# GuyTevet/motion-diffusion-model

Measured on AMD Instinct MI355X. Metric: motions/sec (B=128, T=196, 50-step DDPM), higher is better.
Workload: dtype f16x3 (fp32 operands split into fp16 hi+lo, 3 fp16 MFMA products, fp32 accumulate; everything else fp32); 1 GPU; HumanML3D text2motion, 50-step p_sample_loop with CFG 2.5 (2 denoiser forwards per step), batch=128 per GPU, T=196, 8-layer d=512 trans_enc MDM, random-init weights, cached text embedding; global_batch=128, diffusion_steps=50, parallelism=dp1: batch shards, no data-path collective, all_gather of final samples

## Files before the change

include/mdm_hip.h:

```cpp
#ifndef MDM_HIP_H
#define MDM_HIP_H

#include <stddef.h>
#include <stdint.h>

#ifdef __cplusplus
extern "C" {
#endif

#define MDM_OK 0
#define MDM_EINVAL (-1)
#define MDM_ESTATE (-2)
#define MDM_ENOSPC (-3)
#define MDM_EHIP (-4)
#define MDM_EUNSUPPORTED (-5)

#define MDM_ABI_VERSION 10

typedef struct mdm_model mdm_model_t;

#define MDM_ARCH_TRANS_ENC 0
#define MDM_ARCH_TRANS_DEC 1

typedef struct mdm_config {
// ... 12 lines not shown

int mdm_abi_version(void);
const char* mdm_build_info(void);
const char* mdm_last_error(void);

int mdm_create(const mdm_config_t* cfg, mdm_model_t** out);
void mdm_destroy(mdm_model_t* m);

#define MDM_OPT_SMALL_GEMM_MAX_SEQS 1
#define MDM_OPT_SMALL_GEMM_ROW_TILES 2
#define MDM_OPT_DEC_FUSED_XATTN 3
#define MDM_OPT_DEC_FUSED_SELFATTN 4
#define MDM_OPT_ATTN_DIRECT_OUT 5
#define MDM_OPT_DEC_TIME_TOKEN 6
#define MDM_OPT_ENC_SHARED_LAYER0 7
int mdm_set_option(mdm_model_t* m, int32_t key, int32_t value);
int mdm_get_option(const mdm_model_t* m, int32_t key, int32_t* value);

int mdm_set_time_add(mdm_model_t* m, const float* add_dev, int32_t B);

int mdm_set_weight(mdm_model_t* m, const char* name, const float* dev_ptr, int64_t numel);

size_t mdm_const_bytes(const mdm_model_t* m);
int mdm_prepare(mdm_model_t* m, void* const_ws_dev, size_t const_ws_bytes, void* stream);

int mdm_weights_in_range(mdm_model_t* m, int32_t* in_range, void* stream);

#define MDM_PREC_F32 0
#define MDM_PREC_F16X3 1
int mdm_set_precision(mdm_model_t* m, int32_t mode);
// ... 171 lines not shown
```

motion-diffusion-model_amd/_native.py:

```python
import ctypes as C
import os

_HERE = os.path.dirname(os.path.abspath(__file__))
LIB_NAME = "libmdm_hip.so"
LIB_PATH = os.path.join(_HERE, "csrc", LIB_NAME)
PROBE_LIB_PATH = os.path.join(_HERE, "csrc", "libmdm_hip_probe.so")

MDM_OK = 0
BRANCH_COND, BRANCH_UNCOND, BRANCH_BOTH = 0, 1, 2
ACT_NONE, ACT_GELU, ACT_SILU = 0, 1, 2
PRECISIONS = {"f32": 0, "f16x3": 1}
PROF_CLASSES = ("linear", "attention", "layernorm", "embed", "outproj", "elementwise")

EXPORTED_SYMBOLS = [
    "mdm_abi_version", "mdm_build_info", "mdm_last_error", "mdm_create", "mdm_destroy", "mdm_set_weight", "mdm_const_bytes",
    "mdm_prepare", "mdm_workspace_bytes", "mdm_forward", "mdm_sampler_step", "mdm_randn", "mdm_sample_loop",
    "mdm_linear", "mdm_layernorm", "mdm_attention", "mdm_profile_enable", "mdm_profile_read", "mdm_profile_reset",
    "mdm_set_precision", "mdm_linear_x3", "mdm_linear_x3_scratch_bytes", "mdm_attention_x3", "mdm_attention_x3_scratch_bytes",
    "mdm_recover_from_ric", "mdm_workspace_bytes_dec", "mdm_forward_dec", "mdm_workspace_bytes_dec_loop",
    "mdm_sample_loop_dec", "mdm_weights_in_range", "mdm_set_option", "mdm_get_option", "mdm_set_time_add",
    "mdm_rot6d_to_smpl_joints", "mdm_smpl_workspace_bytes", "mdm_smpl_forward",
    "mdm_eval_workspace_bytes", "mdm_eval_motion_embeddings", "mdm_eval_text_embeddings",
]
PROBE_SYMBOLS = ["mdm_debug_set", "mdm_debug_get", "mdm_linear_f16f6", "mdm_linear_f16f6_scratch_bytes", "mdm_probe_in_proj"]
ABI_VERSION = 10
OPTIONS = {"small_gemm_max_seqs": 1, "small_gemm_row_tiles": 2, "dec_fused_xattn": 3, "dec_fused_selfattn": 4, "attn_direct_out": 5,
           "dec_time_token": 6, "enc_shared_layer0": 7}
ARCH = {"trans_enc": 0, "trans_dec": 1}


class MdmConfig(C.Structure):
    _fields_ = [(n, C.c_int32) for n in ("njoints", "nfeats", "latent_dim", "ff_size", "num_layers", "num_heads",
                                         "clip_dim", "max_len", "mask_frames", "arch", "context_len")]


class MdmSmplModel(C.Structure):
    _fields_ = [(n, C.c_void_p) for n in ("j0", "jdirs", "blend", "weights_t", "sel_blend", "sel_weights_t", "extra_t")] + \
               [("parents", C.POINTER(C.c_int32))] + [(n, C.c_int32) for n in ("J", "V", "n_sel", "n_extra")]


class MdmSmplCall(C.Structure):
    _fields_ = [(n, C.c_int32) for n in ("pose_rep", "glob", "translation", "vertstrans", "n_points", "root_point")] + \
# ... 149 lines not shown
```

motion-diffusion-model_amd/csrc/api_launch.h:

```cpp
#pragma once

namespace {

struct Workspace {
  float *tok, *qkv, *att, *ffn, *cond;
  QkvPlanes qp;
  p16_t *xah, *xal;
  float *stat1, *stat2;
  p16_t *tokh, *tokl;
  p16_t *atth, *attl;
  p16_t *ffnh, *ffnl;
  size_t bytes;
};

QkvPlanes carve_qkv_planes(float* qkv, size_t nseq, size_t S, size_t D, int H) {
  const size_t NKT = (S + 31) / 32, SP = 32 * NKT, plane = nseq * SP * D;
  p16_t* q = reinterpret_cast<p16_t*>(qkv);
  QkvPlanes qp{};
  qp.qh = q; qp.SP = (int)SP; qp.NKT = (int)NKT; qp.H = H;
  if (q != nullptr) { qp.ql = q + plane; qp.kh = q + 2 * plane; qp.kl = q + 3 * plane; qp.vh = q + 4 * plane; qp.vl = q + 5 * plane; }
  return qp;
}

Workspace carve(const mdm_model* m, int nseq, int T, void* base) {
// ... 125 lines not shown
struct X3Call {
  X3Kind kind = X3K_OUT_LN_RES;
  Profiler* pf = nullptr; int prof_cat = MDM_PROF_LINEAR;
  X3Operand a{nullptr, nullptr}; X3Weights w{nullptr, nullptr}; const float* bias = nullptr;
  float* out = nullptr; p16_t* oh = nullptr; p16_t* ol = nullptr; const QkvPlanes* qp = nullptr;
  int M = 0, N = 0, K = 0, S = 0, D = 0;
  int scale_cols = 0; float col_scale = 1.f;
  const float* astat = nullptr; const float* colsum = nullptr;
  X3Operand res{nullptr, nullptr}; const float* rstat = nullptr; const float* rgamma = nullptr; const float* rbeta = nullptr;
  float* ostat = nullptr;
  int parts = 1; float inv_dim = 1.f;
  const float* res_f32 = nullptr; int emb_T = 1, emb_B = 1, emb_nbranch = 1;
  bool small = false;
  X3sShape shape{1};
  int stat_cols = 256;
};
X3Epilogue x3_epilogue(const X3Call& c) {
  X3Epilogue ep{};
  ep.out = c.out; ep.bias = c.bias; ep.res = c.res_f32; ep.resh = c.res.hi; ep.resl = c.res.lo; ep.oh = c.oh; ep.ol = c.ol;
  ep.ld = c.N; ep.scale_cols = c.scale_cols; ep.col_scale = c.col_scale;
  if (c.qp != nullptr) ep.qkv = *c.qp;
  ep.S = c.S; ep.D = c.D;
  ep.astat = c.astat; ep.colsum = c.colsum; ep.rstat = c.rstat; ep.rgamma = c.rgamma; ep.rbeta = c.rbeta; ep.ostat = c.ostat;
  ep.stat_parts = c.parts; ep.inv_dim = c.inv_dim; ep.emb_T = c.emb_T; ep.emb_B = c.emb_B; ep.emb_nbranch = c.emb_nbranch;
  ep.stat_cols = c.stat_cols;
  return ep;
}

#ifdef MDM_PROBES
int g_f6_linear = 0;
// ... 105 lines not shown
  const X3Epilogue ep = x3_epilogue(c);
  const bool in_proj = kind == X3K_IN_PROJ_FOLD || kind == X3K_IN_PROJ_PLAIN;
  if (c.small) {
    const int group_rows = in_proj ? S : (kind == X3K_EMBED ? c.emb_T : M);
    const int rc = launch_gemm_x3s(kind, c.shape, c.a, c.w, ep, M, N, K, group_rows, s);
    if (rc == -1 || rc == -3) return lds_fail(rc, "f16x3 linear (small tiles)");
    if (rc == -2) return fail(MDM_EUNSUPPORTED, "f16x3 linear (small tiles): unsupported shape (K must be 288 or a multiple of 256)");
    return rt_launch_status();
  }
  if (kind == X3K_IN_PROJ_PLAIN) {
    const int rc6 = launch_gemm_x3_qkv(c.a, c.w, ep, M / S, S, c.D, s);
    if (rc6 != 0) return fail(MDM_EUNSUPPORTED, "f16x3 in_proj: launch failed");
    return rt_launch_status();
  }
  const int rpt = (kind == X3K_IN_PROJ_FOLD) ? S : x3_rows_per_tile(M, kind == X3K_EMBED ? c.emb_T : S);
  const int rc = launch_gemm_x3_ln(kind, c.a, c.w, ep, M, N, K, rpt, s);
  if (rc == -1 || rc == -3) return lds_fail(rc, "f16x3 linear");
  if (rc == -2) return fail(MDM_EUNSUPPORTED, "f16x3 linear: unsupported folded-LayerNorm GEMM kind");
  return rt_launch_status();
}

int launch_pack_weights(const float* src, p16_t* hi, p16_t* lo, int N, int K, hipStream_t s, int* overflow = nullptr) {
  if (K % 16 != 0) return fail(MDM_EINVAL, "pack_weights: K must be a multiple of 16");
  const size_t n = x3_packed_weight_elems(N, K) / 8;
  const int grid = (int)std::min<size_t>((n + 255) / 256, 4096);
  MDM_LAUNCH(pack_weight_planes_kernel, dim3(grid), dim3(256), 0, s, src, hi, lo, N, K, overflow);
  return rt_launch_status();
}

int launch_split(const float* src, p16_t* hi, p16_t* lo, size_t n, hipStream_t s) {
  if (n % 4 != 0) return fail(MDM_EINVAL, "split: element count must be a multiple of 4");
// ... 8 lines not shown
```

motion-diffusion-model_amd/csrc/api_runtime.h:

```cpp
#pragma once

namespace {

thread_local std::string g_err;
#ifdef MDM_PROBES
int g_x3_reuse_planes = 0;
int g_f6_reference = 0;
#else
constexpr int g_x3_reuse_planes = 0;
#endif

int fail(int code, const std::string& msg) {
  g_err = msg;
  return code;
}

#ifdef MDM_EMU
inline int rt_launch_status() { return 0; }
inline int rt_copy(void* dst, const void* src, size_t bytes, hipStream_t) { memcpy(dst, src, bytes); return 0; }
template <class K> inline int rt_allow_lds(K, size_t) { return 0; }
#else
inline int rt_launch_status() {
  hipError_t e = hipGetLastError();
  if (e != hipSuccess) return fail(MDM_EHIP, std::string("kernel launch failed: ") + hipGetErrorString(e));
// ... 105 lines not shown
  std::vector<LayerFold> fold;
  struct DecFold { float *w_in, *c_in, *b_in, *w_q, *c_q, *b_q, *w_1, *c_1, *b_1; };
  std::vector<DecFold> dec_fold;
  struct DecPlanes { X3Weights in_proj, out_proj, q, out_proj2, linear1, linear2; };
  std::vector<DecPlanes> dec_planes;
  X3Weights in_planes{nullptr, nullptr};
  int jf_k = 0;
  X3Weights out_planes_f{nullptr, nullptr};
  float *c_out = nullptr, *b_out = nullptr;
  float *wkv_all = nullptr, *bkv_all = nullptr;
  bool lnfold = false;
  X3sOptions x3s;
  int fused_xattn = 3;
  bool fused_selfattn = true;
  bool enc_shared_l0 = true;
  bool attn_direct = false;
  X3Weights out_planes{nullptr, nullptr};
  float* out_bias_pad = nullptr;
  int jf_out = 0;

  const float* W(const std::string& k) const { return w.at(k); }
  const float* L(int layer, const char* suffix) const {
    return w.at((cfg.arch == MDM_ARCH_TRANS_DEC ? "seqTransDecoder.layers." : "seqTransEncoder.layers.") +
                std::to_string(layer) + "." + suffix);
  }
};

namespace {

#ifdef MDM_EMU
// ... 65 lines not shown
```

motion-diffusion-model_amd/csrc/common.h:

```cpp
#pragma once
#ifdef MDM_EMU
#include "hip_emu.h"
#else
#include <hip/hip_runtime.h>
#define MDM_DYN_SMEM(type, name) \
  extern __shared__ __attribute__((aligned(16))) unsigned char mdm_dyn_smem_raw[]; \
  type* name = reinterpret_cast<type*>(mdm_dyn_smem_raw)
#define MDM_LAUNCH(kernel, grid, block, shmem, stream, ...) \
  hipLaunchKernelGGL(kernel, (grid), (block), (shmem), (stream), __VA_ARGS__)
#endif
#include <stdint.h>
#include <type_traits>
#include <utility>

namespace mdm {

typedef float f32x16 __attribute__((ext_vector_type(16)));
typedef short p16x8 __attribute__((ext_vector_type(8)));

constexpr int kWave = 64;

constexpr int kMaxDevices = 64;
inline int rt_device_ordinal() {
#ifdef MDM_EMU
// ... 112 lines not shown
  return __shfl_xor(v, mask, 64);
#endif
}

__device__ __forceinline__ float sum_lanes8(float v) {
#ifdef MDM_EMU
  v += shfl_xor_f32(v, 1);
  v += shfl_xor_f32(v, 2);
  v += shfl_xor_f32(v, 4);
  return v;
#else
  v += __builtin_bit_cast(float, __builtin_amdgcn_update_dpp(0, __builtin_bit_cast(int, v), 0xB1, 0xF, 0xF, true));
  v += __builtin_bit_cast(float, __builtin_amdgcn_update_dpp(0, __builtin_bit_cast(int, v), 0x4E, 0xF, 0xF, true));
  v += __builtin_bit_cast(float, __builtin_amdgcn_update_dpp(0, __builtin_bit_cast(int, v), 0x141, 0xF, 0xF, true));
  return v;
#endif
}

template <int KT>
__device__ __forceinline__ bool key_valid_bits(const uint32_t* __restrict__ w, int row, int lead) {
  const int f = row - lead;
  uint32_t word;
  if (f >= 0) word = w[KT];
  else word = (KT > 0) ? w[KT > 0 ? KT - 1 : 0] : 0xffffffffu;
  return (word >> (f & 31)) & 1u;
}

__device__ __forceinline__ float4 ld4(const float* p) { return *reinterpret_cast<const float4*>(p); }
__device__ __forceinline__ void st4(float* p, float4 v) { *reinterpret_cast<float4*>(p) = v; }
__device__ __forceinline__ float4 zero4() { return make_float4(0.f, 0.f, 0.f, 0.f); }
// ... 215 lines not shown
  split2_p16(v.x, v.y, h01, l01);
  split2_p16(v.z, v.w, h23, l23);
  clip_store8(hi_w, off, u32x2{h01, h23});
  clip_store8(lo_w, off, u32x2{l01, l23});
}
__device__ __forceinline__ void clip_load8_async(u32x2& dst, const ClipWin& w, uint32_t off) {
#ifdef MDM_EMU
  static const uint32_t zeros[2] = {0u, 0u};
  const bool in = off < w.bytes && off + 8 <= w.bytes;
  emu::vm_issue(&dst, in ? static_cast<const void*>(w.base + off) : static_cast<const void*>(zeros), 8, true);
#else
  asm volatile("buffer_load_dwordx2 %0, %1, %2, 0 offen" : "=&v"(dst) : "v"(off), "s"(w.d) : "memory");
#endif
}

__device__ __forceinline__ void wg_barrier() {
#ifdef MDM_EMU
  emu::lgkm_wait(0);
  emu::block_barrier();
#else
  __builtin_amdgcn_s_waitcnt(0xC07F);
  __builtin_amdgcn_s_barrier();
#endif
}
__device__ __forceinline__ void wg_barrier_nodrain() {
#ifdef MDM_EMU
  emu::block_barrier();
#else
  __builtin_amdgcn_s_barrier();
#endif
// ... 79 lines not shown
```

motion-diffusion-model_amd/csrc/decoder.h:

```cpp
#pragma once

namespace {
struct DecWorkspace {
  float *tok, *qkv, *att, *ffn, *mem, *kv, *proj;
  float *stat[2];
  p16_t *xh[2], *xl[2];
  p16_t *atth, *attl, *ffnh, *ffnl;
  QkvPlanes qp;
  float *out;
  float *kv_text;
  float *kv_time;
  float *time_rows;
  float *o_text;
  float *o_time;
  size_t bytes;
};
DecWorkspace carve_dec(const mdm_model* m, int nseq, int S, int ntok, int B, void* base, int nsteps = 0, int pred_len = 0) {
  const size_t D = m->cfg.latent_dim, FF = m->cfg.ff_size, M = (size_t)nseq * S, Mm = (size_t)nseq * ntok;
  size_t off = 0;
  auto take = [&](size_t floats) {
    size_t o = off;
    off += align_up(floats * sizeof(float), 256);
    return base ? reinterpret_cast<float*>(static_cast<char*>(base) + o) : nullptr;
  };
// ... 128 lines not shown

struct DecLayer {
  int l; p16_t *Xh, *Xl, *Yh, *Yl; float *sX, *sY;
  X3Operand X() const { return X3Operand{Xh, Xl}; }
  X3Operand Y() const { return X3Operand{Yh, Yl}; }
};
struct DecStack {
  mdm_model_t* m; const DecWorkspace& ws; const DecHoist& hz; hipStream_t s; Profiler* pf;
  const int32_t* text_lengths; const int32_t* len;
  int B, nbranch, nseq, S, ntok, D, H, FF, M;
  bool small; X3sShape shape; int scols, parts; float inv_dim, qscale;

  X3Call LN(X3Kind kind, X3Operand a, X3Weights w, const float* bias, int rows, int N, int K) const {
    X3Call c; c.kind = kind; c.pf = pf; c.a = a; c.w = w; c.bias = bias; c.M = rows; c.N = N; c.K = K; c.S = S; c.D = D;
    c.small = small; c.shape = shape; c.stat_cols = scols; c.parts = parts; c.inv_dim = inv_dim;
    return c;
  }
  SelfAttnArgs seqhead_args() const {
    SelfAttnArgs a{};
    a.qscale = qscale; a.lead = 0; a.B = B; a.oh = ws.atth; a.ol = ws.attl;
    a.M = M; a.S = S; a.D = D; a.H = H; a.stat_parts = parts; a.stat_cols = scols; a.inv_dim = inv_dim; a.acc_scale = kX3AccScale;
    return a;
  }

  int self_attention(const DecLayer& y, DecSelfForm form, bool share0) const {
    const int l = y.l;
    const mdm_model::DecFold& F = m->dec_fold[l];
    const mdm_model::DecPlanes& P = m->dec_planes[l];
    const int M0 = (share0 && l == 0) ? B * S : M;
    const float* b_in = l == 0 ? m->L(l, "self_attn.in_proj_bias") : F.b_in;
// ... 258 lines not shown
```

motion-diffusion-model_amd/csrc/encoder.h:

```cpp
#pragma once

namespace {

int embed_frames_x3(mdm_model* m, const Workspace& ws, const float* x, int B, int T, int nbranch, hipStream_t s, const CondTokArgs& ct) {
  const int D = m->cfg.latent_dim, KP = m->jf_k;
  ProfScope ps(&m->prof, MDM_PROF_EMBED, 2.0 * B * T * (double)D * m->jf, s);
  p16_t* ph = reinterpret_cast<p16_t*>(ws.ffn);
  p16_t* pl = ph + (size_t)B * T * KP;
  MDM_LAUNCH(pose_planes_cond_kernel, dim3(((T + 31) / 32) * (KP / 32) * B + nbranch * B), dim3(256), 0, s, x, ph, pl, T, m->jf, KP, B, ct);
  if (int rc = rt_launch_status()) return rc;
  X3Call c;
  c.kind = X3K_EMBED; c.prof_cat = MDM_PROF_EMBED;
  c.a = X3Operand{ph, pl}; c.w = m->in_planes; c.bias = m->W("input_process.poseEmbedding.bias");
  c.oh = ws.tokh; c.ol = ws.tokl; c.M = B * T; c.N = D; c.K = KP; c.S = T + 1; c.D = D;
  c.res_f32 = m->W("sequence_pos_encoder.pe");
  c.emb_T = T; c.emb_B = B; c.emb_nbranch = nbranch;
  c.small = use_small_gemm(m, nbranch * B, T + 1) && KP == 288;
  c.shape = x3s_shape(m->x3s, nbranch * B);
  return launch_x3_ln(c, s);
}
inline bool use_embed_x3(const mdm_model* m, int T) {
  return m->precision == MDM_PREC_F16X3 &&
         (T + 1 <= X3_TM || (use_small_gemm(m, 1, T + 1) && m->jf_k == 288));
}
// ... 22 lines not shown
                                false, s)) return rc;
  ProfScope ps(&m->prof, MDM_PROF_ELEMENTWISE, 0.0, s);
  MDM_LAUNCH(cond_token_kernel, dim3(nbranch * B), dim3(128), 0, s, ws.tok, cond_emb, m->W("embed_text.bias"),
             (const float*)m->time_table, timesteps, t_uniform, m->W("sequence_pos_encoder.pe"), B, S, D, uncond_from_branch,
             (int)m->cfg.max_len, x3 ? ws.tokh : (p16_t*)nullptr, x3 ? ws.tokl : (p16_t*)nullptr, m->time_add);
  return rt_launch_status();
}

X3Call enc_ln_call(mdm_model* m, int nseq, int S) {
  const int D = m->cfg.latent_dim;
  X3Call c; c.M = nseq * S; c.S = S; c.D = D; c.inv_dim = 1.0f / (float)D;
  c.small = use_small_gemm(m, nseq, S);
  c.shape = x3s_shape(m->x3s, nseq);
  c.stat_cols = c.small ? X3S_TN : 256;
  c.parts = (D + c.stat_cols - 1) / c.stat_cols;
  return c;
}

int encoder(mdm_model* m, const Workspace& ws, int nseq, int B, int S, const int* lengths, hipStream_t s) {
  Profiler* pf = &m->prof;
  const int D = m->cfg.latent_dim, FF = m->cfg.ff_size, H = m->cfg.num_heads, M = nseq * S;
  const float qscale = 1.0f / sqrtf((float)(D / H));
  if (m->precision == MDM_PREC_F16X3 && m->lnfold && (S <= X3_TM || use_small_gemm(m, nseq, S))) {
    const X3Operand xb{ws.tokh, ws.tokl}, xa{ws.xah, ws.xal}, attp{ws.atth, ws.attl}, ffnp{ws.ffnh, ws.ffnl};
    const X3Call stack = enc_ln_call(m, nseq, S);
    const bool small = stack.small;
    auto LN = [&](X3Kind kind, X3Operand a, X3Weights w, const float* bias, int N, int K) {
      X3Call c = stack; c.kind = kind; c.pf = pf; c.a = a; c.w = w; c.bias = bias; c.N = N; c.K = K;
      return c;
    };
// ... 96 lines not shown
```

motion-diffusion-model_amd/csrc/gemm_x3.h:

```cpp
#pragma once
#include "attention_x3.h"
#include "common.h"
#include "gemm_f32.h"

namespace mdm {

constexpr int X3_TM = 224, X3_BK = 32;
__host__ __device__ constexpr int x3_swz(int q) { return (((q ^ (q >> 1)) & 1) << 1) | (q >> 1); }
static_assert(x3_swz(0) == 0 && x3_swz(1) == 2 && x3_swz(2) == 3 && x3_swz(3) == 1, "A-stage swizzle permutation");
constexpr int X3_NWAVE = 8;
constexpr int X3_TN = 32 * X3_NWAVE;
constexpr int X3_MSUB = X3_TM / 32;
constexpr int X3_A_BYTES = X3_TM * X3_BK * 2;
constexpr int X3_A_STAGE = 2 * X3_A_BYTES;
constexpr int X3_A_RING = 2;
constexpr int X3_PIPE_RING = 4;
constexpr int X3M_WAIT_WS = 7, X3M_WAIT_MID = 11;
constexpr int x3_patch_base(int ring) { return ring * X3_A_STAGE; }
constexpr int X3_PATCH_BYTES = 8 * 32 * 4;
constexpr int X3_TAB_BYTES = X3_TM * 8;
constexpr int x3_tab_base(int ring) { return x3_patch_base(ring) + X3_NWAVE * X3_PATCH_BYTES; }
constexpr int X3_RAW_BYTES = 7 * 1024;
constexpr int x3_raw_base(int ring) { return x3_tab_base(ring) + 2 * X3_TAB_BYTES; }
constexpr int x3_part_base(int ring) { return x3_raw_base(ring) + 2 * X3_RAW_BYTES; }
// ... 104 lines not shown
  int k;
  uint32_t off[X3_A_PIECES];
};

enum : unsigned {
  X3_OUT_F32 = 1u << 0,
  X3_OUT_PLANES = 1u << 1,
  X3_OUT_QKV = 1u << 2,
  X3_FOLD = 1u << 3,
  X3_OSTAT = 1u << 4,
  X3_EMBED = 1u << 5,
  X3_T16 = 1u << 6,
  X3_F6 = 1u << 7,
  X3_PIPE = 1u << 8,
  X3_PAIR = 1u << 9,
};
template <int ACT, int RES, unsigned FLAGS>
__global__ __launch_bounds__(64 * X3_NWAVE, 2) void gemm_x3_kernel(X3Operand A, X3Weights W, X3Epilogue ep, int M, int N, int K,
                                                                   int rows_per_tile, int tiles_n, int total) {
  MDM_DYN_SMEM(unsigned char, lds);
  constexpr bool OUT_F32 = (FLAGS & X3_OUT_F32) != 0, OUT_PLANES = (FLAGS & X3_OUT_PLANES) != 0, OUT_QKV = (FLAGS & X3_OUT_QKV) != 0;
  constexpr bool FOLD = (FLAGS & X3_FOLD) != 0, OSTAT = (FLAGS & X3_OSTAT) != 0, EMBED = (FLAGS & X3_EMBED) != 0;
  constexpr bool T16 = (FLAGS & X3_T16) != 0, F6 = (FLAGS & X3_F6) != 0, PIPE = (FLAGS & X3_PIPE) != 0, PAIR = (FLAGS & X3_PAIR) != 0;
  static_assert(FLAGS < (X3_PAIR << 1), "unknown flag");
  static_assert((int)OUT_F32 + (int)OUT_PLANES + (int)OUT_QKV == 1, "exactly one output form");
  static_assert(RES >= 0 && RES <= 3 && !(OUT_QKV && RES != 0), "in_proj has no residual");
  static_assert(!(FOLD && RES == 3), "one (mean, rstd) table: of the A rows or of the residual rows");
  static_assert(!OSTAT || OUT_PLANES, "row statistics are written next to the planes they describe");
  static_assert(!EMBED || (OUT_PLANES && RES == 1 && !PIPE), "InputProcess: fp32 positional rows, planes out, step-synchronous loop");
  static_assert(!PIPE || (T16 && !F6), "the pipelined k-loop exists for 208-row (T16) tiles");
  static_assert(!F6 || (!T16 && OUT_F32 && !FOLD && !OSTAT), "the f16f6 k-loop: 224-row tiles, plain fp32-out epilogues");
  static_assert(!PAIR || (PIPE && OUT_QKV && !FOLD), "the paired tile: layer 0's in_proj (no folded LayerNorm) on the pipelined loop");
  constexpr int RINGN = PIPE ? X3_PIPE_RING : X3_A_RING;
  constexpr int NT32 = T16 ? X3_MSUB - 1 : X3_MSUB;
  constexpr int NROUNDS = 4 * NT32 + (T16 ? 2 : 0);
  using Cursor = X3Cursor;

  const int tid = threadIdx.x;
  const int lane = tid & 63;
#ifdef MDM_EMU
  const int wid = tid >> 6;
#else
  const int wid = __builtin_amdgcn_readfirstlane(tid >> 6);
#endif
  const int r = lane & 31, h = lane >> 5;
  const int nk = K / X3_BK;
  const int gstride = (int)gridDim.x;
// ... 86 lines not shown
  {
    int m0f, n0f;
    tile_origin(v, m0f, n0f);
    if constexpr (FOLD || RES == 3) stats_dma(m0f, 0);
    cvec_dma(n0f, 0);
  }
  p16x8 wh[2], wl[2], wnh[2], wnl[2];
  p16x8 wsh[4] = {}, wsl[4] = {};
  uint32_t wso = 0;
  uint32_t wtile = 0;
  auto aim_w_tile = [&]() {
    int m0w, n0w;
    tile_origin(wv, m0w, n0w);
    wtile = (uint32_t)((n0w >> 5) + wid) * (uint32_t)wk16 * 512u;
  };
  const uint32_t lane_wo = (uint32_t)((lane >> 5) * 512 + ((lane & 15) + 32 * ((lane >> 4) & 1)) * 8);
  auto aim_w = [&]() { wso = wtile + (uint32_t)wkk * 1024u + lane_wo; };
  auto advance_w = [&]() {
    if (++wkk == nk) {
      wkk = 0;
      if (wv + gstride < total) { wv += gstride; aim_w_tile(); }
    }
  };
  auto load_w_half = [&](int c, auto q_tag) __attribute__((always_inline)) {
    constexpr int q = decltype(q_tag)::value;
    const uint32_t o = wso + 128u * (uint32_t)c;
    gload16_refill(wsh[q], W.hi + o);
    gload16_refill(wsl[q], W.lo + o);
  };
  auto wait_all_slots = [&]() __attribute__((always_inline)) {
    vmem_wait<0>(wsh[0], wsl[0], wsh[1], wsl[1], wsh[2], wsl[2], wsh[3], wsl[3]);
  };
  int gs = 0;
  if constexpr (PIPE) {
#pragma unroll
    for (int st = 0; st < 3; ++st) {
#pragma unroll
      for (int i = 0; i < X3_A_PIECES; ++i) piece_a(ca, i, st);
      advance_a(ca);
    }
    aim_w_tile();
// ... 92 lines not shown
        constexpr int PAR = decltype(par_tag)::value, W0 = 2 * PAR, W1 = 2 * PAR + 1;
        const uint32_t cur = (uint32_t)gs & 3u, nxt = (uint32_t)(gs + 1) & 3u, fill = (uint32_t)(gs + 3) & 3u;
        vmem_wait<X3M_WAIT_WS>(wsh[W0], wsl[W0], wsh[W1], wsl[W1]);
        static_for<NE>([&](auto e_tag) __attribute__((always_inline)) {
          constexpr int e = decltype(e_tag)::value;
          if constexpr (e + DEPTH < NE) issue_reads(std::integral_constant<int, e + DEPTH>{}, cur);
          else issue_reads(std::integral_constant<int, e + DEPTH - NE>{}, nxt);
          if constexpr (e == XB) {
            vmem_wait<X3M_WAIT_MID>(wsh[W0], wsl[W0], wsh[W1], wsl[W1]);
            sched_fence();
            wg_barrier_nodrain();
            sched_fence();
          }
          lds_wait<2 * DEPTH>(ah[slot(e)], al[slot(e)]);
          sched_fence();
#pragma unroll
          for (int c = 0; c < 2; ++c) accm_[e][c] = mfma16_p16(al[slot(e)], wsh[W0 + c], accm_[e][c]);
#pragma unroll
          for (int c = 0; c < 2; ++c) accm_[e][c] = mfma16_p16(ah[slot(e)], wsl[W0 + c], accm_[e][c]);
#pragma unroll
          for (int c = 0; c < 2; ++c) accm_[e][c] = mfma16_p16(ah[slot(e)], wsh[W0 + c], accm_[e][c]);
          sched_fence();
          if constexpr (e >= XB && e < XB + X3_A_PIECES) piece_a(ca, e - XB, (int)fill);
          sched_fence();
        });
        aim_w();
        load_w_half(0, std::integral_constant<int, W0>{});
        load_w_half(1, std::integral_constant<int, W1>{});
        advance_w();
        advance_a(ca);
        ++gs;
      };
      static_for<DEPTH>([&](auto d_tag) __attribute__((always_inline)) { issue_reads(d_tag, (uint32_t)gs & 3u); });
      for (int kt = 0; kt < nk; kt += 2) {
        pipe_step(std::integral_constant<int, 0>{});
        if (kt == 0 && v + gstride < total) {
// ... 286 lines not shown
              const int tok = 32 * t + 8 * g + prow;
              v4 = finish4(v4, st);
              if constexpr (PAIR) {
                if (tok < ep.S) split4_store(dh + tok * AX_HD, dl + tok * AX_HD, v4);
                if ((unsigned)(tok - 1) < (unsigned)ep.S) {
                  const int tok2 = tok == ep.S ? 0 : tok;
                  split4_store(dh + pq + tok2 * AX_HD, dl + pq + tok2 * AX_HD, v4);
                }
              } else {
                if (t < X3_MSUB - 1 || tok < ep.S) split4_store(dh + tok * AX_HD, dl + tok * AX_HD, v4);
              }
            }
          });
        }
      }
    } else {
      constexpr bool HAS_RES = RES != 0;
      constexpr bool RES_PLANES = RES == 2 || RES == 3;
      static_assert(!(EMBED && RES_PLANES), "the EMBED epilogue takes an fp32 residual");
      constexpr bool CLIP_OUT = OUT_PLANES && !EMBED;
      const uint32_t pitch2 = (uint32_t)ep.ld * 2u;
      const uint32_t voff0 = n4 < N ? ((uint32_t)prow * (uint32_t)ep.ld + (uint32_t)n4) * 2u : CLIP_OFF;
      ClipWin w_oh = {}, w_ol = {}, w_rh = {}, w_rl = {};
      {
        int m0_e = m0;
#ifndef MDM_EMU
        asm volatile("" : "+s"(m0_e));
#endif
        const size_t row0 = (size_t)m0_e * ep.ld;
        if constexpr (CLIP_OUT) {
// ... 168 lines not shown
  MDM_LAUNCH(kfn, dim3(grid), dim3(64 * X3_NWAVE), x3_lds_bytes(LN, RINGN), stream, A, W, ep, M, N, K, rpt, tiles_n, total);
  return 0;
}

enum X3Kind : int {
  X3K_IN_PROJ_FOLD = 0,
  X3K_OUT_PROJ_L0 = 1,
  X3K_OUT_LN_RES = 2,
  X3K_LINEAR1_GELU = 3,
  X3K_FOLD_F32 = 4,
  X3K_EMBED = 5,
  X3K_IN_PROJ_PLAIN = 6,
};
template <unsigned TILE>
inline int launch_gemm_x3_ln_t(X3Kind kind, const X3Operand& A, const X3Weights& W, const X3Epilogue& ep, int M, int N,
                                   int K, int rpt, hipStream_t s) {
  switch (kind) {
    case X3K_IN_PROJ_FOLD: return launch_gemm_x3_w<ACT_NONE,  0, X3_OUT_QKV | X3_FOLD | TILE>(A, W, ep, M, N, K, rpt, s);
    case X3K_OUT_PROJ_L0: return launch_gemm_x3_w<ACT_NONE,  2, X3_OUT_PLANES | X3_OSTAT | TILE>(A, W, ep, M, N, K, rpt, s);
    case X3K_OUT_LN_RES: return launch_gemm_x3_w<ACT_NONE,  3, X3_OUT_PLANES | X3_OSTAT | TILE>(A, W, ep, M, N, K, rpt, s);
    case X3K_LINEAR1_GELU: return launch_gemm_x3_w<ACT_GELU,  0, X3_OUT_PLANES | X3_FOLD | TILE>(A, W, ep, M, N, K, rpt, s);
    case X3K_FOLD_F32: return launch_gemm_x3_w<ACT_NONE,  0, X3_OUT_F32 | X3_FOLD | TILE>(A, W, ep, M, N, K, rpt, s);
    case X3K_EMBED:
      return launch_gemm_x3_w<ACT_NONE,  1, X3_OUT_PLANES | X3_EMBED | (TILE & X3_T16)>(A, W, ep, M, N, K, rpt, s);
    default: return -2;
  }
}
inline int launch_gemm_x3_ln(X3Kind kind, const X3Operand& A, const X3Weights& W, const X3Epilogue& ep, int M, int N,
                                 int K, int rpt, hipStream_t s) {
  if (rpt <= X3_TM - 16) {
    if (kind != X3K_EMBED && (K / X3_BK) % 2 == 0) return launch_gemm_x3_ln_t<X3_T16 | X3_PIPE>(kind, A, W, ep, M, N, K, rpt, s);
    return launch_gemm_x3_ln_t<X3_T16>(kind, A, W, ep, M, N, K, rpt, s);
  }
  return launch_gemm_x3_ln_t<0u>(kind, A, W, ep, M, N, K, rpt, s);
}

inline int launch_gemm_x3(const X3Operand& A, const X3Weights& W, const X3Epilogue& ep, int M, int N, int K, int act,
                              int seq_len, hipStream_t s) {
  const bool res = ep.res != nullptr, f32 = ep.out != nullptr, pl = ep.oh != nullptr;
  const int rpt = x3_rows_per_tile(M, seq_len);
  if (ep.resh != nullptr) {
    if (act == ACT_NONE && !res && f32 && !pl) return launch_gemm_x3_w<ACT_NONE,  2, X3_OUT_F32>(A, W, ep, M, N, K, rpt, s);
    return -2;
  }
  if (act == ACT_NONE && !res && f32 && !pl) return launch_gemm_x3_w<ACT_NONE,  0, X3_OUT_F32>(A, W, ep, M, N, K, rpt, s);
  if (act == ACT_NONE && res && f32 && !pl) return launch_gemm_x3_w<ACT_NONE,  1, X3_OUT_F32>(A, W, ep, M, N, K, rpt, s);
  if (act == ACT_GELU && !res && !f32 && pl) return launch_gemm_x3_w<ACT_GELU,  0, X3_OUT_PLANES>(A, W, ep, M, N, K, rpt, s);
  if (act == ACT_GELU && !res && f32 && !pl) return launch_gemm_x3_w<ACT_GELU,  0, X3_OUT_F32>(A, W, ep, M, N, K, rpt, s);
  if (act == ACT_GELU && res && f32 && !pl) return launch_gemm_x3_w<ACT_GELU,  1, X3_OUT_F32>(A, W, ep, M, N, K, rpt, s);
// ... 37 lines not shown
```

motion-diffusion-model_amd/csrc/mdm_api.hip:

```cpp
#include "../../include/mdm_hip.h"
#ifdef MDM_PROBES
#include "../../include/mdm_hip_probe.h"
#endif

#include <algorithm>
#include <cmath>
#include <cstdio>
#include <cstring>
#include <map>
#include <mutex>
#include <new>
#include <string>
#include <vector>

#include "attention_x3.h"
#include "attention_long.h"
#include "attention_f32.h"
#include "common.h"
#include "elementwise.h"
#include "gemm_f32.h"
#include "gemm_x3.h"
#include "gemm_x3s.h"
#include "xattn_block.h"
#include "selfattn_block.h"
// ... 121 lines not shown
      return MDM_OK;
    case MDM_OPT_ATTN_DIRECT_OUT:
      if (value != 0 && value != 1) return fail(MDM_EINVAL, "mdm_set_option: MDM_OPT_ATTN_DIRECT_OUT must be 0 or 1");
      m->attn_direct = value != 0;
      return MDM_OK;
    case MDM_OPT_DEC_TIME_TOKEN:
      if (value != 0 && value != 1) return fail(MDM_EINVAL, "mdm_set_option: MDM_OPT_DEC_TIME_TOKEN must be 0 or 1");
      if (value == 1 && (m->cfg.arch != MDM_ARCH_TRANS_DEC || m->cfg.context_len != 1))
        return fail(MDM_EINVAL, "mdm_set_option: MDM_OPT_DEC_TIME_TOKEN needs a trans_dec model created with context_len = 1 (the class-token row)");
      m->dec_time_token = value != 0;
      return MDM_OK;
    case MDM_OPT_ENC_SHARED_LAYER0:
      if (value != 0 && value != 1) return fail(MDM_EINVAL, "mdm_set_option: MDM_OPT_ENC_SHARED_LAYER0 must be 0 or 1");
      m->enc_shared_l0 = value != 0;
      return MDM_OK;
    default:
      return fail(MDM_EINVAL, "mdm_set_option: unknown key " + std::to_string(key));
  }
}

int mdm_set_time_add(mdm_model_t* m, const float* add_dev, int32_t B) {
  if (m == nullptr) return fail(MDM_EINVAL, "mdm_set_time_add: null model");
  if (add_dev != nullptr && B <= 0) return fail(MDM_EINVAL, "mdm_set_time_add: B must be >= 1");
  m->time_add_next = add_dev;
  m->time_add_B = add_dev != nullptr ? B : 0;
  return MDM_OK;
}

int mdm_get_option(const mdm_model_t* m, int32_t key, int32_t* value) {
  if (m == nullptr || value == nullptr) return fail(MDM_EINVAL, "mdm_get_option: null argument");
  switch (key) {
    case MDM_OPT_SMALL_GEMM_MAX_SEQS: *value = m->x3s.max_seqs; return MDM_OK;
    case MDM_OPT_SMALL_GEMM_ROW_TILES: *value = m->x3s.row_tiles; return MDM_OK;
    case MDM_OPT_DEC_FUSED_XATTN: *value = m->fused_xattn; return MDM_OK;
    case MDM_OPT_DEC_FUSED_SELFATTN: *value = m->fused_selfattn ? 1 : 0; return MDM_OK;
    case MDM_OPT_ATTN_DIRECT_OUT: *value = m->attn_direct ? 1 : 0; return MDM_OK;
    case MDM_OPT_DEC_TIME_TOKEN: *value = m->dec_time_token ? 1 : 0; return MDM_OK;
    case MDM_OPT_ENC_SHARED_LAYER0: *value = m->enc_shared_l0 ? 1 : 0; return MDM_OK;
    default: return fail(MDM_EINVAL, "mdm_get_option: unknown key " + std::to_string(key));
  }
}

int mdm_set_weight(mdm_model_t* m, const char* name, const float* dev_ptr, int64_t numel) {
  if (m == nullptr || name == nullptr || dev_ptr == nullptr) return fail(MDM_EINVAL, "mdm_set_weight: null argument");
  auto it = m->expect.find(name);
  if (it == m->expect.end()) return fail(MDM_EINVAL, std::string("unexpected state-dict key: ") + name);
  if (it->second != numel)
    return fail(MDM_EINVAL, std::string("size mismatch for ") + name + ": expected " + std::to_string(it->second) +
                                " elements, got " + std::to_string(numel));
  if ((reinterpret_cast<uintptr_t>(dev_ptr) & 15) != 0) return fail(MDM_EINVAL, std::string(name) + ": pointer must be 16-byte aligned");
  m->w[name] = dev_ptr;
  m->prepared = false;
  return MDM_OK;
// ... 922 lines not shown
```

Measured before the change: 401.8 motions/s.

## Add transposed-accumulator row epilogue for pipelined plane-writing f16x3 GEMMs

Adds a ROWACC variant of the pipelined f16x3 GEMM that swaps the MFMA operands, so each lane's accumulators hold consecutive output columns of one row. The epilogue can then load residual planes and store hi/lo planes as 16-byte vectors through clipped buffer ops, with prefetched residual loads. LayerNorm partial statistics are reduced with permlane16/32 swaps. It applies by default to out_proj, out-LN-residual and linear1-GELU when N%8==0, and is controlled by a new option. In exchange it reorders weight-fragment loads and adds a second epilogue path, which brings correctness risk and register pressure.

```diff
diff --git a/include/mdm_hip.h b/include/mdm_hip.h
--- a/include/mdm_hip.h
+++ b/include/mdm_hip.h
@@ -50,6 +50,7 @@
 #define MDM_OPT_ATTN_DIRECT_OUT 5
 #define MDM_OPT_DEC_TIME_TOKEN 6
 #define MDM_OPT_ENC_SHARED_LAYER0 7
+#define MDM_OPT_GEMM_ROW_EPILOGUE 8
 int mdm_set_option(mdm_model_t* m, int32_t key, int32_t value);
 int mdm_get_option(const mdm_model_t* m, int32_t key, int32_t* value);
 
diff --git a/motion-diffusion-model_amd/_native.py b/motion-diffusion-model_amd/_native.py
--- a/motion-diffusion-model_amd/_native.py
+++ b/motion-diffusion-model_amd/_native.py
@@ -25,7 +25,7 @@
 PROBE_SYMBOLS = ["mdm_debug_set", "mdm_debug_get", "mdm_linear_f16f6", "mdm_linear_f16f6_scratch_bytes", "mdm_probe_in_proj"]
 ABI_VERSION = 10
 OPTIONS = {"small_gemm_max_seqs": 1, "small_gemm_row_tiles": 2, "dec_fused_xattn": 3, "dec_fused_selfattn": 4, "attn_direct_out": 5,
-           "dec_time_token": 6, "enc_shared_layer0": 7}
+           "dec_time_token": 6, "enc_shared_layer0": 7, "gemm_row_epilogue": 8}
 ARCH = {"trans_enc": 0, "trans_dec": 1}
 
 
diff --git a/motion-diffusion-model_amd/csrc/api_launch.h b/motion-diffusion-model_amd/csrc/api_launch.h
--- a/motion-diffusion-model_amd/csrc/api_launch.h
+++ b/motion-diffusion-model_amd/csrc/api_launch.h
@@ -163,6 +163,7 @@
   bool small = false;
   X3sShape shape{1};
   int stat_cols = 256;
+  bool row_epilogue = true;
 };
 X3Epilogue x3_epilogue(const X3Call& c) {
   X3Epilogue ep{};
@@ -298,7 +299,7 @@
     return rt_launch_status();
   }
   const int rpt = (kind == X3K_IN_PROJ_FOLD) ? S : x3_rows_per_tile(M, kind == X3K_EMBED ? c.emb_T : S);
-  const int rc = launch_gemm_x3_ln(kind, c.a, c.w, ep, M, N, K, rpt, s);
+  const int rc = launch_gemm_x3_ln(kind, c.a, c.w, ep, M, N, K, rpt, s, c.row_epilogue);
   if (rc == -1 || rc == -3) return lds_fail(rc, "f16x3 linear");
   if (rc == -2) return fail(MDM_EUNSUPPORTED, "f16x3 linear: unsupported folded-LayerNorm GEMM kind");
   return rt_launch_status();
diff --git a/motion-diffusion-model_amd/csrc/api_runtime.h b/motion-diffusion-model_amd/csrc/api_runtime.h
--- a/motion-diffusion-model_amd/csrc/api_runtime.h
+++ b/motion-diffusion-model_amd/csrc/api_runtime.h
@@ -143,6 +143,7 @@
   int fused_xattn = 3;
   bool fused_selfattn = true;
   bool enc_shared_l0 = true;
+  bool gemm_row_epilogue = true;
   bool attn_direct = false;
   X3Weights out_planes{nullptr, nullptr};
   float* out_bias_pad = nullptr;
diff --git a/motion-diffusion-model_amd/csrc/common.h b/motion-diffusion-model_amd/csrc/common.h
--- a/motion-diffusion-model_amd/csrc/common.h
+++ b/motion-diffusion-model_amd/csrc/common.h
@@ -150,6 +150,23 @@
   v += __builtin_bit_cast(float, __builtin_amdgcn_update_dpp(0, __builtin_bit_cast(int, v), 0x4E, 0xF, 0xF, true));
   v += __builtin_bit_cast(float, __builtin_amdgcn_update_dpp(0, __builtin_bit_cast(int, v), 0x141, 0xF, 0xF, true));
   return v;
+#endif
+}
+
+__device__ __forceinline__ float sum_lanes_x16_x32(float v) {
+  uint32_t x = __builtin_bit_cast(uint32_t, v), y = x;
+#ifdef MDM_EMU
+  emu::permlane16_swap(x, y);
+  v = __builtin_bit_cast(float, x) + __builtin_bit_cast(float, y);
+  x = y = __builtin_bit_cast(uint32_t, v);
+  emu::permlane32_swap(x, y);
+  return __builtin_bit_cast(float, x) + __builtin_bit_cast(float, y);
+#else
+  const auto s16 = __builtin_amdgcn_permlane16_swap(x, y, false, false);
+  v = __builtin_bit_cast(float, (uint32_t)s16[0]) + __builtin_bit_cast(float, (uint32_t)s16[1]);
+  x = y = __builtin_bit_cast(uint32_t, v);
+  const auto s32 = __builtin_amdgcn_permlane32_swap(x, y, false, false);
+  return __builtin_bit_cast(float, (uint32_t)s32[0]) + __builtin_bit_cast(float, (uint32_t)s32[1]);
 #endif
 }
 
@@ -395,6 +412,39 @@
 #endif
 }
 
+__device__ __forceinline__ void clip_store16(const ClipWin& w, uint32_t off, u32x4 v) {
+#ifdef MDM_EMU
+  if (off < w.bytes && off + 16 <= w.bytes) *reinterpret_cast<u32x4*>(w.base + off) = v;
+#else
+  asm volatile("buffer_store_dwordx4 %0, %1, %2, 0 offen\n\ts_nop 1" : : "v"(v), "v"(off), "s"(w.d) : "memory");
+#endif
+}
+__device__ __forceinline__ void split8_store_clip(const ClipWin& hi_w, const ClipWin& lo_w, uint32_t off, float4 a, float4 b) {
+  uint32_t h01, l01, h23, l23, h45, l45, h67, l67;
+  split2_p16(a.x, a.y, h01, l01);
+  split2_p16(a.z, a.w, h23, l23);
+  split2_p16(b.x, b.y, h45, l45);
+  split2_p16(b.z, b.w, h67, l67);
+  clip_store16(hi_w, off, u32x4{h01, h23, h45, h67});
+  clip_store16(lo_w, off, u32x4{l01, l23, l45, l67});
+}
+__device__ __forceinline__ void clip_load16_async(u32x4& dst, const ClipWin& w, uint32_t off) {
+#ifdef MDM_EMU
+  static const uint32_t zeros[4] = {0u, 0u, 0u, 0u};
+  const bool in = off < w.bytes && off + 16 <= w.bytes;
+  emu::vm_issue(&dst, in ? static_cast<const void*>(w.base + off) : static_cast<const void*>(zeros), 16, true);
+#else
+  asm volatile("buffer_load_dwordx4 %0, %1, %2, 0 offen" : "=&v"(dst) : "v"(off), "s"(w.d) : "memory");
+#endif
+}
+template <int N> __device__ __forceinline__ void vmem_wait(u32x4& a, u32x4& b) {
+#ifdef MDM_EMU
+  emu::vm_wait(N);
+#else
+  asm volatile("s_waitcnt vmcnt(%2)" : "+v"(a), "+v"(b) : "i"(N) : "memory");
+#endif
+}
+
 __device__ __forceinline__ void wg_barrier() {
 #ifdef MDM_EMU
   emu::lgkm_wait(0);
diff --git a/motion-diffusion-model_amd/csrc/decoder.h b/motion-diffusion-model_amd/csrc/decoder.h
--- a/motion-diffusion-model_amd/csrc/decoder.h
+++ b/motion-diffusion-model_amd/csrc/decoder.h
@@ -166,6 +166,7 @@
   X3Call LN(X3Kind kind, X3Operand a, X3Weights w, const float* bias, int rows, int N, int K) const {
     X3Call c; c.kind = kind; c.pf = pf; c.a = a; c.w = w; c.bias = bias; c.M = rows; c.N = N; c.K = K; c.S = S; c.D = D;
     c.small = small; c.shape = shape; c.stat_cols = scols; c.parts = parts; c.inv_dim = inv_dim;
+    c.row_epilogue = m->gemm_row_epilogue;
     return c;
   }
   SelfAttnArgs seqhead_args() const {
diff --git a/motion-diffusion-model_amd/csrc/encoder.h b/motion-diffusion-model_amd/csrc/encoder.h
--- a/motion-diffusion-model_amd/csrc/encoder.h
+++ b/motion-diffusion-model_amd/csrc/encoder.h
@@ -60,6 +60,7 @@
   c.shape = x3s_shape(m->x3s, nseq);
   c.stat_cols = c.small ? X3S_TN : 256;
   c.parts = (D + c.stat_cols - 1) / c.stat_cols;
+  c.row_epilogue = m->gemm_row_epilogue;
   return c;
 }
 
diff --git a/motion-diffusion-model_amd/csrc/gemm_x3.h b/motion-diffusion-model_amd/csrc/gemm_x3.h
--- a/motion-diffusion-model_amd/csrc/gemm_x3.h
+++ b/motion-diffusion-model_amd/csrc/gemm_x3.h
@@ -142,6 +142,7 @@
   X3_F6 = 1u << 7,
   X3_PIPE = 1u << 8,
   X3_PAIR = 1u << 9,
+  X3_ROWACC = 1u << 10,
 };
 template <int ACT, int RES, unsigned FLAGS>
 __global__ __launch_bounds__(64 * X3_NWAVE, 2) void gemm_x3_kernel(X3Operand A, X3Weights W, X3Epilogue ep, int M, int N, int K,
@@ -150,7 +151,8 @@
   constexpr bool OUT_F32 = (FLAGS & X3_OUT_F32) != 0, OUT_PLANES = (FLAGS & X3_OUT_PLANES) != 0, OUT_QKV = (FLAGS & X3_OUT_QKV) != 0;
   constexpr bool FOLD = (FLAGS & X3_FOLD) != 0, OSTAT = (FLAGS & X3_OSTAT) != 0, EMBED = (FLAGS & X3_EMBED) != 0;
   constexpr bool T16 = (FLAGS & X3_T16) != 0, F6 = (FLAGS & X3_F6) != 0, PIPE = (FLAGS & X3_PIPE) != 0, PAIR = (FLAGS & X3_PAIR) != 0;
-  static_assert(FLAGS < (X3_PAIR << 1), "unknown flag");
+  constexpr bool ROWACC = (FLAGS & X3_ROWACC) != 0;
+  static_assert(FLAGS < (X3_ROWACC << 1), "unknown flag");
   static_assert((int)OUT_F32 + (int)OUT_PLANES + (int)OUT_QKV == 1, "exactly one output form");
   static_assert(RES >= 0 && RES <= 3 && !(OUT_QKV && RES != 0), "in_proj has no residual");
   static_assert(!(FOLD && RES == 3), "one (mean, rstd) table: of the A rows or of the residual rows");
@@ -159,6 +161,8 @@
   static_assert(!PIPE || (T16 && !F6), "the pipelined k-loop exists for 208-row (T16) tiles");
   static_assert(!F6 || (!T16 && OUT_F32 && !FOLD && !OSTAT), "the f16f6 k-loop: 224-row tiles, plain fp32-out epilogues");
   static_assert(!PAIR || (PIPE && OUT_QKV && !FOLD), "the paired tile: layer 0's in_proj (no folded LayerNorm) on the pipelined loop");
+  static_assert(!ROWACC || (PIPE && OUT_PLANES && RES != 1 && !x3_has_col_scale(ACT, RES)),
+                "transposed accumulators: the plane-writing GEMMs of the pipelined loop (no fp32 residual, no column scale)");
   constexpr int RINGN = PIPE ? X3_PIPE_RING : X3_A_RING;
   constexpr int NT32 = T16 ? X3_MSUB - 1 : X3_MSUB;
   constexpr int NROUNDS = 4 * NT32 + (T16 ? 2 : 0);
@@ -275,7 +279,9 @@
     tile_origin(wv, m0w, n0w);
     wtile = (uint32_t)((n0w >> 5) + wid) * (uint32_t)wk16 * 512u;
   };
-  const uint32_t lane_wo = (uint32_t)((lane >> 5) * 512 + ((lane & 15) + 32 * ((lane >> 4) & 1)) * 8);
+  constexpr uint32_t W_HALF = ROWACC ? 32u : 128u;
+  const int wcol = ROWACC ? 8 * ((lane & 15) >> 2) + (lane & 3) : (lane & 15);
+  const uint32_t lane_wo = (uint32_t)((lane >> 5) * 512 + (wcol + 32 * ((lane >> 4) & 1)) * 8);
   auto aim_w = [&]() { wso = wtile + (uint32_t)wkk * 1024u + lane_wo; };
   auto advance_w = [&]() {
     if (++wkk == nk) {
@@ -285,7 +291,7 @@
   };
   auto load_w_half = [&](int c, auto q_tag) __attribute__((always_inline)) {
     constexpr int q = decltype(q_tag)::value;
-    const uint32_t o = wso + 128u * (uint32_t)c;
+    const uint32_t o = wso + W_HALF * (uint32_t)c;
     gload16_refill(wsh[q], W.hi + o);
     gload16_refill(wsl[q], W.lo + o);
   };
@@ -408,12 +414,16 @@
           }
           lds_wait<2 * DEPTH>(ah[slot(e)], al[slot(e)]);
           sched_fence();
-#pragma unroll
-          for (int c = 0; c < 2; ++c) accm_[e][c] = mfma16_p16(al[slot(e)], wsh[W0 + c], accm_[e][c]);
-#pragma unroll
-          for (int c = 0; c < 2; ++c) accm_[e][c] = mfma16_p16(ah[slot(e)], wsl[W0 + c], accm_[e][c]);
-#pragma unroll
-          for (int c = 0; c < 2; ++c) accm_[e][c] = mfma16_p16(ah[slot(e)], wsh[W0 + c], accm_[e][c]);
+          auto mm = [](const p16x8& a, const p16x8& w, f32x4 acc) __attribute__((always_inline)) {
+            if constexpr (ROWACC) return mfma16_p16(w, a, acc);
+            else return mfma16_p16(a, w, acc);
+          };
+#pragma unroll
+          for (int c = 0; c < 2; ++c) accm_[e][c] = mm(al[slot(e)], wsh[W0 + c], accm_[e][c]);
+#pragma unroll
+          for (int c = 0; c < 2; ++c) accm_[e][c] = mm(ah[slot(e)], wsl[W0 + c], accm_[e][c]);
+#pragma unroll
+          for (int c = 0; c < 2; ++c) accm_[e][c] = mm(ah[slot(e)], wsh[W0 + c], accm_[e][c]);
           sched_fence();
           if constexpr (e >= XB && e < XB + X3_A_PIECES) piece_a(ca, e - XB, (int)fill);
           sched_fence();
@@ -730,6 +740,118 @@
           });
         }
       }
+    } else if constexpr (ROWACC) {
+      const int row16 = lane_e & 15, q16 = lane_e >> 4;
+      const int cl8 = wid * 32 + 8 * q16;
+      const int n8 = ncol0 + 8 * q16;
+      const float accs = ep.acc_scale;
+      float4 bb8[2], c8[2] = {zero4(), zero4()}, g8[2] = {zero4(), zero4()};
+#pragma unroll
+      for (int hc = 0; hc < 2; ++hc) {
+        bb8[hc] = ld4(cvec + cl8 + 4 * hc);
+        if constexpr (FOLD) c8[hc] = ld4(cvec + 256 + cl8 + 4 * hc);
+        if constexpr (RES == 3) {
+          g8[hc] = ld4(cvec + 512 + cl8 + 4 * hc);
+          const float4 be4 = ld4(cvec + 768 + cl8 + 4 * hc);
+          bb8[hc] = make_float4(bb8[hc].x + be4.x, bb8[hc].y + be4.y, bb8[hc].z + be4.z, bb8[hc].w + be4.w);
+        }
+      }
+      auto finish4r = [&](f32x4 a, float2 st, const float4& c4, const float4& bb4) __attribute__((always_inline)) {
+        float4 v4 = make_float4(a[0], a[1], a[2], a[3]);
+        v4.x *= accs; v4.y *= accs; v4.z *= accs; v4.w *= accs;
+        if constexpr (FOLD) {
+          v4.x = st.y * (v4.x - st.x * c4.x) + bb4.x; v4.y = st.y * (v4.y - st.x * c4.y) + bb4.y;
+          v4.z = st.y * (v4.z - st.x * c4.z) + bb4.z; v4.w = st.y * (v4.w - st.x * c4.w) + bb4.w;
+        } else {
+          v4.x += bb4.x; v4.y += bb4.y; v4.z += bb4.z; v4.w += bb4.w;
+        }
+        if (ACT == ACT_GELU) { v4.x = gelu_erf_fast(v4.x); v4.y = gelu_erf_fast(v4.y); v4.z = gelu_erf_fast(v4.z); v4.w = gelu_erf_fast(v4.w); }
+        else if (ACT == ACT_SILU) { v4.x = silu(v4.x); v4.y = silu(v4.y); v4.z = silu(v4.z); v4.w = silu(v4.w); }
+        return v4;
+      };
+      auto add_res4 = [&](float4& v4, uint32_t a0, uint32_t b0, uint32_t a1, uint32_t b1, float2 st, const float4& g4) __attribute__((always_inline)) {
+        const float c0 = RES == 3 ? -st.x : 0.f;
+        const float d0 = f16_half_plus<0>(b0, f16_half_plus<0>(a0, c0));
+        const float d1 = f16_half_plus<1>(b0, f16_half_plus<1>(a0, c0));
+        const float d2 = f16_half_plus<0>(b1, f16_half_plus<0>(a1, c0));
+        const float d3 = f16_half_plus<1>(b1, f16_half_plus<1>(a1, c0));
+        if constexpr (RES == 3) {
+          v4.x = fmaf(d0, st.y * g4.x, v4.x); v4.y = fmaf(d1, st.y * g4.y, v4.y);
+          v4.z = fmaf(d2, st.y * g4.z, v4.z); v4.w = fmaf(d3, st.y * g4.w, v4.w);
+        } else {
+          v4.x += d0; v4.y += d1; v4.z += d2; v4.w += d3;
+        }
+      };
+      auto row_stats16 = [&](auto s_tag) __attribute__((always_inline)) {
+        constexpr int s = decltype(s_tag)::value;
+        if constexpr (LN_TABS && s < NS16) return stab[16 * s + row16];
+        else return make_float2(0.f, 1.f);
+      };
+      constexpr bool HAS_RES = RES != 0;
+      const uint32_t pitch2 = (uint32_t)ep.ld * 2u;
+      const uint32_t voff0 = n8 < N ? ((uint32_t)row16 * (uint32_t)ep.ld + (uint32_t)n8) * 2u : CLIP_OFF;
+      ClipWin w_oh = {}, w_ol = {}, w_rh = {}, w_rl = {};
+      {
+        int m0_e = m0;
+#ifndef MDM_EMU
+        asm volatile("" : "+s"(m0_e));
+#endif
+        const size_t row0 = (size_t)m0_e * ep.ld;
+        const uint32_t bytes = (uint32_t)(m_end - m0_e) * pitch2;
+        w_oh = clip_win(ep.oh + row0, bytes);
+        w_ol = clip_win(ep.ol + row0, bytes);
+        if constexpr (HAS_RES) {
+          const uint32_t rbytes = (uint32_t)min(M - m0_e, X3_TM) * pitch2;
+          w_rh = clip_win(ep.resh + row0, rbytes);
+          w_rl = clip_win(ep.resl + row0, rbytes);
+        }
+      }
+      constexpr int RR = (RES == 3) ? 3 : 4;
+      u32x4 rh[RR], rl[RR];
+      auto res_issue = [&](auto s_tag) __attribute__((always_inline)) {
+        constexpr int s = decltype(s_tag)::value;
+        if constexpr (HAS_RES && s < NS16) {
+          const uint32_t o = voff0 + (uint32_t)(16 * s) * pitch2;
+          clip_load16_async(rh[s % RR], w_rh, o);
+          clip_load16_async(rl[s % RR], w_rl, o);
+        }
+      };
+      static_for<RR - 1>([&](auto s_tag) __attribute__((always_inline)) { res_issue(s_tag); });
+      float2* part = reinterpret_cast<float2*>(lds + x3_part_base(RINGN)) + wid * X3_TM;
+      float2 st_cur = row_stats16(std::integral_constant<int, 0>{});
+      static_for<NS16>([&](auto s_tag) __attribute__((always_inline)) {
+        constexpr int s = decltype(s_tag)::value;
+        if constexpr (HAS_RES) {
+          res_issue(std::integral_constant<int, s + RR - 1>{});
+          constexpr int ahead = (NS16 - 1 - s) < (RR - 1) ? (NS16 - 1 - s) : (RR - 1);
+          vmem_wait<2 * ahead>(rh[s % RR], rl[s % RR]);
+        }
+        const float2 st = st_cur;
+        st_cur = row_stats16(std::integral_constant<int, s + 1>{});
+        float4 va = finish4r(accm_[s][0], st, c8[0], bb8[0]);
+        float4 vb = finish4r(accm_[s][1], st, c8[1], bb8[1]);
+        if constexpr (HAS_RES) {
+          const u32x4 a = rh[s % RR], b = rl[s % RR];
+          add_res4(va, a[0], b[0], a[1], b[1], st, g8[0]);
+          add_res4(vb, a[2], b[2], a[3], b[3], st, g8[1]);
+        }
+        if constexpr (OSTAT) {
+          const float s1 = sum_lanes_x16_x32(((va.x + va.y) + (va.z + va.w)) + ((vb.x + vb.y) + (vb.z + vb.w)));
+          const float mw = s1 * (1.0f / 32.0f);
+          auto sq4 = [&](const float4& v4) __attribute__((always_inline)) {
+            const float dx = v4.x - mw, dy = v4.y - mw, dz = v4.z - mw, dw = v4.w - mw;
+            float q = (dx * dx + dy * dy) + (dz * dz + dw * dw);
+#ifndef MDM_EMU
+            asm volatile("" : "+v"(q));
+#endif
+            return q;
+          };
+          const float qa = sq4(va), qb = sq4(vb);
+          const float m2 = sum_lanes_x16_x32(qa + qb);
+          if (q16 == 0) part[16 * s + row16] = make_float2(s1, m2);
+        }
+        split8_store_clip(w_oh, w_ol, voff0 + (uint32_t)(16 * s) * pitch2, va, vb);
+      });
     } else {
       constexpr bool HAS_RES = RES != 0;
       constexpr bool RES_PLANES = RES == 2 || RES == 3;
@@ -928,7 +1050,18 @@
 };
 template <unsigned TILE>
 inline int launch_gemm_x3_ln_t(X3Kind kind, const X3Operand& A, const X3Weights& W, const X3Epilogue& ep, int M, int N,
-                                   int K, int rpt, hipStream_t s) {
+                                   int K, int rpt, hipStream_t s, bool row_epilogue) {
+  if constexpr ((TILE & X3_PIPE) != 0) {
+    if (row_epilogue && N % 8 == 0) {
+      constexpr unsigned ROW = TILE | X3_ROWACC;
+      switch (kind) {
+        case X3K_OUT_PROJ_L0: return launch_gemm_x3_w<ACT_NONE,  2, X3_OUT_PLANES | X3_OSTAT | ROW>(A, W, ep, M, N, K, rpt, s);
+        case X3K_OUT_LN_RES: return launch_gemm_x3_w<ACT_NONE,  3, X3_OUT_PLANES | X3_OSTAT | ROW>(A, W, ep, M, N, K, rpt, s);
+        case X3K_LINEAR1_GELU: return launch_gemm_x3_w<ACT_GELU,  0, X3_OUT_PLANES | X3_FOLD | ROW>(A, W, ep, M, N, K, rpt, s);
+        default: break;
+      }
+    }
+  }
   switch (kind) {
     case X3K_IN_PROJ_FOLD: return launch_gemm_x3_w<ACT_NONE,  0, X3_OUT_QKV | X3_FOLD | TILE>(A, W, ep, M, N, K, rpt, s);
     case X3K_OUT_PROJ_L0: return launch_gemm_x3_w<ACT_NONE,  2, X3_OUT_PLANES | X3_OSTAT | TILE>(A, W, ep, M, N, K, rpt, s);
@@ -941,12 +1074,12 @@
   }
 }
 inline int launch_gemm_x3_ln(X3Kind kind, const X3Operand& A, const X3Weights& W, const X3Epilogue& ep, int M, int N,
-                                 int K, int rpt, hipStream_t s) {
+                                 int K, int rpt, hipStream_t s, bool row_epilogue) {
   if (rpt <= X3_TM - 16) {
-    if (kind != X3K_EMBED && (K / X3_BK) % 2 == 0) return launch_gemm_x3_ln_t<X3_T16 | X3_PIPE>(kind, A, W, ep, M, N, K, rpt, s);
-    return launch_gemm_x3_ln_t<X3_T16>(kind, A, W, ep, M, N, K, rpt, s);
+    if (kind != X3K_EMBED && (K / X3_BK) % 2 == 0) return launch_gemm_x3_ln_t<X3_T16 | X3_PIPE>(kind, A, W, ep, M, N, K, rpt, s, row_epilogue);
+    return launch_gemm_x3_ln_t<X3_T16>(kind, A, W, ep, M, N, K, rpt, s, row_epilogue);
   }
-  return launch_gemm_x3_ln_t<0u>(kind, A, W, ep, M, N, K, rpt, s);
+  return launch_gemm_x3_ln_t<0u>(kind, A, W, ep, M, N, K, rpt, s, row_epilogue);
 }
 
 inline int launch_gemm_x3(const X3Operand& A, const X3Weights& W, const X3Epilogue& ep, int M, int N, int K, int act,
diff --git a/motion-diffusion-model_amd/csrc/mdm_api.hip b/motion-diffusion-model_amd/csrc/mdm_api.hip
--- a/motion-diffusion-model_amd/csrc/mdm_api.hip
+++ b/motion-diffusion-model_amd/csrc/mdm_api.hip
@@ -159,6 +159,10 @@
       if (value != 0 && value != 1) return fail(MDM_EINVAL, "mdm_set_option: MDM_OPT_ENC_SHARED_LAYER0 must be 0 or 1");
       m->enc_shared_l0 = value != 0;
       return MDM_OK;
+    case MDM_OPT_GEMM_ROW_EPILOGUE:
+      if (value != 0 && value != 1) return fail(MDM_EINVAL, "mdm_set_option: MDM_OPT_GEMM_ROW_EPILOGUE must be 0 or 1");
+      m->gemm_row_epilogue = value != 0;
+      return MDM_OK;
     default:
       return fail(MDM_EINVAL, "mdm_set_option: unknown key " + std::to_string(key));
   }
@@ -182,6 +186,7 @@
     case MDM_OPT_ATTN_DIRECT_OUT: *value = m->attn_direct ? 1 : 0; return MDM_OK;
     case MDM_OPT_DEC_TIME_TOKEN: *value = m->dec_time_token ? 1 : 0; return MDM_OK;
     case MDM_OPT_ENC_SHARED_LAYER0: *value = m->enc_shared_l0 ? 1 : 0; return MDM_OK;
+    case MDM_OPT_GEMM_ROW_EPILOGUE: *value = m->gemm_row_epilogue ? 1 : 0; return MDM_OK;
     default: return fail(MDM_EINVAL, "mdm_get_option: unknown key " + std::to_string(key));
   }
 }
```

Result: no change. 399.6 motions/s (-0.5%).
